# SudhirNikam/cobrix

Hardware: AMD Instinct MI355X
Metric: decoded input GB/s + records/s, fixed-len COMP-3 mix, 1-8 MI355X; % HBM peak (higher is better)
Workload: dtype u8; 1 GPU; SYN200: fixed-length 200-byte EBCDIC records, numeric mix (COMP, COMP-3, zoned DISPLAY overpunch, IBM COMP-2, cp037 X(18)) -- BASELINE config C2; records_per_gpu=50000000, input_bytes_per_gpu=10000000000, job_input_bytes=10000000000, output_columns=28, parallelism=dp1, string_layout=Arrow string views (16 B views + long payloads, one pass), occurs_layout=Arrow lists (present elements only), inputs_resident_in_hbm=True

## Files before the change

cobrix_amd/csrc/cbx_capi.hip:

```cpp
#include <hip/hip_runtime.h>

#include <algorithm>
#include <cstdio>
#include <cstring>
#include <functional>
#include <string>
#include <vector>

#include "cbx_kernels.hip"
#include "cbx_select.h"
#include "cbx_text.h"
#include "cbx_hier.h"
#include "cbx_walk.h"
#include "cbx_chain.h"
#include "cbx_filter.h"
#include "cbx_gather.h"

using namespace cbx;

static thread_local std::string g_err;

static int fail(int code, const std::string& msg) {
    g_err = msg;
    return code;
}

#define HIP_CHECK(x)                                                                   \
    do {                                                                               \
        hipError_t e_ = (x);                                                           \
        if (e_ != hipSuccess) return fail(CBX_E_HIP, std::string(#x) + ": " + hipGetErrorString(e_)); \
    } while (0)

struct cbx_plan {
    std::vector<cbx_field> hfields;
    std::vector<Field> dfields_h;
    std::vector<cbx_array> harrays;
    struct OpSet {
        std::vector<Window> win;
        std::vector<NumOp> nops;
        std::vector<Batch> batches;
        std::vector<StrOp> sops;
        std::vector<GenOp> gops;
        Window* d_win = nullptr;
        NumOp* d_nops = nullptr;
        Batch* d_batches = nullptr;
        StrOp* d_sops = nullptr;
        GenOp* d_gops = nullptr;
        int max_str_items = 0;
        bool has_runs = false;
    } cset, wset;
    bool contig_ok = true;
    int str_stage = 16;
    bool view_staged = false;
    cbx_plan_options opts;
    int n_columns = 0;
    int seg_col = -1;
    int max_pitch = 0;
    int n_seq = 0;
    std::vector<DeferSeq> hdefer;
    std::vector<int32_t> col_is_string;
    std::vector<int32_t> col_slots;
    std::vector<int32_t> col_max_bytes;
    bool view = false;
    bool packed = false;
    std::vector<int32_t> segid_cols;
    std::vector<ListOp> lops;
    ListOp* d_lops = nullptr;
    int32_t* d_list_len = nullptr;  int64_t list_len_cap = 0;
    int32_t* d_list_flag = nullptr; int64_t list_flag_cap = 0;
    Field* d_fields = nullptr;
    DeferSeq* d_defer = nullptr;
    uint64_t* d_defer_bits = nullptr;
    int64_t defer_bits_cap = 0;
    cbx_array* d_arrays = nullptr;
    cbx_segment_map* d_segmap = nullptr;
    uint32_t* d_lut = nullptr;
    DevColumn* d_cols = nullptr;
    std::vector<DevColumn> h_cols;
    std::vector<NumCall> h_ncall;
    std::vector<StrCall> h_scall;
    NumCall* d_ncall = nullptr;
    StrCall* d_scall = nullptr;
    size_t ncall_cap = 0, scall_cap = 0;
    std::vector<int32_t> seq_field, seq_slot;
    std::vector<int64_t> seq_tile_cap;
    std::vector<SeqCall> h_seqcall;
    std::vector<int64_t> h_seq_scratch;
    SeqCall* d_seqcall = nullptr;
    uint32_t* d_str_tot = nullptr;  int64_t str_tot_cap = 0;
    int64_t* d_str_excl = nullptr;  int64_t str_excl_cap = 0;
    int64_t* d_block_sums = nullptr; int64_t block_sums_cap = 0;
    uint32_t* d_local = nullptr;    int64_t local_cap = 0;
    uint8_t* d_scratch = nullptr;   int64_t scratch_cap = 0;
    uint64_t* d_stamps = nullptr;
    int64_t jit_min = 262144;
    bool jit_tried[4 * kPre + 5] = {};
    hipFunction_t jit_fn[4 * kPre + 5] = {};
    bool jit_coop[4 * kPre + 5] = {};
    int rec_extent = 0;
    std::string jit_error;
    int last_kind = 0;
    int32_t* d_status = nullptr;
    int num_cus = 256;
    bool walk = false;
    int32_t walk_root = 0, walk_var = 0, walk_n_handlers = 0, walk_depth = 1, walk_max_rec = 0;
    cbx_walk_node* d_wnodes = nullptr;
    std::vector<cbx_walk_node> h_wnodes;
    std::vector<cbx_walk_array> h_warr;
    bool walk_jit_tried = false;
    hipFunction_t walk_jit_fn = nullptr;
    bool chain_jit_tried = false;
    hipFunction_t chain_jit_fn[5] = {};
    bool last_chain_jit = false;
    cbx_walk_array* d_warr = nullptr;
    cbx_walk_handler* d_whand = nullptr;
    int64_t* d_wslot_base = nullptr;
    int64_t* d_wtile_bytes = nullptr;
    const int64_t* d_rec_base = nullptr;
    const int32_t* d_odo = nullptr;
    int64_t odo_pitch = 0;
    const int64_t* d_dep_seed = nullptr;
    int64_t seed_pitch = 0;
    int32_t seed_root = -1;
    int64_t n_str_slots = 0;
    uint32_t* d_wcursor = nullptr; int64_t wcursor_cap = 0;
    int64_t* d_wvbase = nullptr;
    int32_t* d_wvcol = nullptr;
    int32_t* d_wvslot = nullptr;
    int32_t n_vslots = 0;
    int32_t fid_col = -1, rid_col = -1;
    cbx_plan* pipe_peer = nullptr;
    hipEvent_t pipe_done = nullptr;
    int pipe_count_bpc = 0, pipe_decode_bpc = 0;
    bool profiling = false;
    std::vector<hipEvent_t> ev_pool;
    struct CallEvents { hipEvent_t e[3]; };
    std::vector<CallEvents> ev_calls;
    float flt_ms[3] = {0.f, 0.f, 0.f};
    bool direct_ok = false;
    std::string direct_why;
    std::vector<GatherOp> gather_ops;
    GatherOp* d_gather = nullptr;
// ... 190 lines not shown
        while (e1 < els.size() && std::max(hi, els[e1].eo + els[e1].size) - lo <= wmax && items + (els[e1].str ? 1 : 0) <= kMaxStrItems) {
            hi = std::max(hi, els[e1].eo + els[e1].size);
            items += els[e1].str ? 1 : 0;
            e1++;
        }
        push_window(P, P->wset, std::vector<Elem>(els.begin() + e0, els.begin() + e1), lo, hi, false, {});
        e0 = e1;
    }
    if (!big.empty() || !gen.empty()) push_window(P, P->wset, big, 0, 0, true, gen);
}

template <typename T>
static int upload_vec(T** dst, const std::vector<T>& v) { return upload(dst, v.data(), v.size()); }

static int upload_set(cbx_plan::OpSet& S) {
    int r;
    if ((r = upload_vec(&S.d_win, S.win)) || (r = upload_vec(&S.d_nops, S.nops)) || (r = upload_vec(&S.d_batches, S.batches)) ||
        (r = upload_vec(&S.d_sops, S.sops)) ||
        (r = upload_vec(&S.d_gops, S.gops)))
        return r;
    return CBX_OK;
}

static void free_set(cbx_plan::OpSet& S) {
    (void)hipFree(S.d_win); (void)hipFree(S.d_nops); (void)hipFree(S.d_batches); (void)hipFree(S.d_sops); (void)hipFree(S.d_gops);
}

extern "C" int cbx_plan_create(const cbx_field* fields, int32_t n_fields, const cbx_array* arrays,
                               int32_t n_arrays, const cbx_plan_options* opts, cbx_plan** out_plan) {
    if (!fields || n_fields <= 0 || !opts || !out_plan || n_arrays < 0 || (n_arrays > 0 && !arrays))
        return fail(CBX_E_ARGUMENT, "cbx_plan_create: invalid arguments");
    cbx_plan* P = new cbx_plan();
    P->opts = *opts;
    P->jit_min = opts->jit_min_records < 0 ? -1 : (opts->jit_min_records == 0 ? 262144 : opts->jit_min_records);
    if (const char* e = getenv("CBX_JIT"))
        if (e[0] == '0') P->jit_min = -1;
    P->n_columns = opts->n_columns;
    if (opts->string_views < 0 || opts->string_views > 2)
        { delete P; return fail(CBX_E_ARGUMENT, "cbx_plan_create: string_views must be 0, 1 or 2"); }
    P->view = opts->string_views == 1;
    P->packed = opts->string_views == 2;
    if (P->n_columns <= 0) { delete P; return fail(CBX_E_ARGUMENT, "cbx_plan_create: n_columns must be positive"); }
    P->hfields.assign(fields, fields + n_fields);
    if (n_arrays) P->harrays.assign(arrays, arrays + n_arrays);
    P->col_is_string.assign(P->n_columns, 0);
    P->col_slots.assign(P->n_columns, 1);
    P->col_max_bytes.assign(P->n_columns, 0);

    int lut_max = 1;
    for (int i = 0; i < 256; i++) lut_max = std::max(lut_max, (int)((opts->lut[i] >> 24) & 3));

    for (int i = 0; i < n_fields; i++) {
        const cbx_field& f = fields[i];
        const std::string fi = "field " + std::to_string(i);
        if (f.n_dims < 0 || f.n_dims > CBX_MAX_DIMS) { delete P; return fail(CBX_E_ARGUMENT, fi + ": bad n_dims"); }
        for (int k = 0; k < f.n_dims; k++)
            if (f.dim_count[k] <= 0 || f.dim_array[k] < 0 || f.dim_array[k] >= n_arrays) {
                delete P; return fail(CBX_E_ARGUMENT, fi + ": bad dimension");
            }
        Field d = make_field(f);
        if (f.column < 0 || f.column >= P->n_columns) { delete P; return fail(CBX_E_ARGUMENT, fi + ": bad column"); }
        if (!is_generated(d) && (f.size <= 0 || f.offset < 0)) { delete P; return fail(CBX_E_ARGUMENT, fi + ": bad offset/size"); }
        if (!(f.kind >= CBX_K_STRING && f.kind <= CBX_K_UTF16_LE)) { delete P; return fail(CBX_E_ARGUMENT, fi + ": unknown kind"); }
        if (f.kind == CBX_K_BINARY && f.size > 16) { delete P; return fail(CBX_E_UNSUPPORTED, fi + ": binary wider than 16 bytes"); }
        if (f.kind == CBX_K_ASCII_NUM && (f.size > kAsciiNumMax || f.scale < 0 || f.scale > 100 || f.scale_factor < -100 ||
                                          f.scale_factor > 100)) {
            delete P; return fail(CBX_E_UNSUPPORTED, fi + ": ASCII DISPLAY number wider than 64 bytes");
        }
        if ((f.out_type == CBX_O_DEC64 || f.out_type == CBX_O_DEC128) && (f.out_precision < 1 || f.out_precision > 38)) {
            delete P; return fail(CBX_E_UNSUPPORTED, fi + ": decimal precision outside 1..38");
        }
        if (d.variant == V_STRING) {
            if (f.kind == CBX_K_STRING) d.max_utf8 = lut_max;
            d.seq = P->n_seq;
            P->n_seq += d.n_slots;
            for (int sl = 0; sl < d.n_slots; sl++) {
                P->seq_field.push_back(i);
                P->seq_slot.push_back(sl);
                P->seq_tile_cap.push_back(((int64_t)kWave * f.size * d.max_utf8 + 15) & ~(int64_t)15);
            }
            P->col_max_bytes[f.column] = f.size * d.max_utf8;
        } else if ((d.variant == V_ZONED16 || d.variant == V_GENERIC) && !(f.flags & CBX_F_LIST)) {
            d.defer = (int)P->hdefer.size();
            for (int s = 0; s < d.n_slots; s++) P->hdefer.push_back(DeferSeq{i, s});
        }
        P->dfields_h.push_back(d);
        P->col_is_string[f.column] = is_string_out(f.out_type);
        P->col_slots[f.column] = d.n_slots;
    }
    for (int ai = 0; ai < n_arrays; ai++) {
        const cbx_array& ar = arrays[ai];
        if (ar.dependee >= n_fields || ar.max_count <= 0) { delete P; return fail(CBX_E_ARGUMENT, "array " + std::to_string(ai) + ": bad descriptor"); }
        if (ar.offsets_column >= P->n_columns || (ar.offsets_column >= 0 && (ar.dependee < 0 || ar.n_dims != 0)))
            { delete P; return fail(CBX_E_ARGUMENT, "array " + std::to_string(ai) + ": list layout needs a top-level OCCURS DEPENDING ON"); }
        if (ar.dependee >= 0) {
            const cbx_field& df = fields[ar.dependee];
            if (!(df.flags & CBX_F_INTEGRAL) || df.n_dims != 0 || df.precision > 18)
                { delete P; return fail(CBX_E_UNSUPPORTED, "array " + std::to_string(ai) + ": DEPENDING ON source must be a non-array integral field"); }
        }
    }
    for (int ai = 0; ai < n_arrays; ai++)
        for (int i = 0; i < n_fields; i++) {
            const cbx_field& f = fields[i];
            if (!(f.flags & CBX_F_LIST) || (f.n_dims == 1 && f.dim_array[0] != ai)) continue;
            if (f.n_dims != 1 || arrays[ai].offsets_column < 0 || is_string_out(f.out_type) || f.segment != arrays[ai].segment)
                { delete P; return fail(CBX_E_ARGUMENT, "field " + std::to_string(i) + ": CBX_F_LIST needs a numeric element of a list-layout array in its segment"); }
            ListOp lo{};
            const int16_t none[CBX_MAX_DIMS] = {0, 0, 0, 0};
            lo.op = make_numop(P->dfields_h[i], 0, f.offset, none, none, 0);
            lo.field = i;
            lo.array = ai;
            lo.stride = f.dim_stride[0];
            P->lops.push_back(lo);
        }
    for (ListOp& lo : P->lops) {
        lo.elem_lo = lo.op.eo;
        for (const ListOp& o : P->lops)
            if (o.array == lo.array) lo.elem_lo = std::min(lo.elem_lo, o.op.eo);
    }
    if ((int)P->lops.size() != (int)std::count_if(fields, fields + n_fields, [](const cbx_field& f) { return (f.flags & CBX_F_LIST) != 0; }))
        { delete P; return fail(CBX_E_ARGUMENT, "CBX_F_LIST field outside a list-layout array"); }
    P->seg_col = opts->segment_column;
    if (P->seg_col >= P->n_columns) { delete P; return fail(CBX_E_ARGUMENT, "bad segment column"); }

    int wmax = opts->window_bytes > 0 ? opts->window_bytes : 256;
    if (wmax > kMaxWindowBytes) wmax = kMaxWindowBytes;
    build_contig(P);
    build_windowed(P, wmax);
    int slots = 0;
    if (P->view || P->packed) P->str_stage = 0;
    for (const Field& d : P->dfields_h) {
        if (d.variant != V_STRING) continue;
        const bool fast = d.size <= kStrFastBytes && (d.kind == CBX_K_STRING || d.kind == CBX_K_STRING_ASCII);
        if ((P->view || P->packed) && fast) {
            if (d.max_utf8 > 1 || getenv("CBX_STR_NO_SHIFT")) slots = std::max(slots, kWave * str_lane_slot(d.size, d.max_utf8));
        } else {
            P->str_stage = std::max(P->str_stage, kWave * d.size * d.max_utf8);
            P->view_staged |= P->view;
        }
    }
    P->str_stage = std::min(P->str_stage, kStrStageBytes);
    for (const cbx_field& f : P->hfields) {
        if (f.flags & CBX_F_LIST) continue;
        int64_t e = (int64_t)f.offset + f.size;
        for (int k = 0; k < f.n_dims; k++) e += (int64_t)(f.dim_count[k] - 1) * f.dim_stride[k];
        if (f.kind != CBX_K_RECORD_ID && f.kind != CBX_K_FILE_ID)
            P->rec_extent = std::max(P->rec_extent, (int)std::min<int64_t>(e, 1 << 30));
    }
    P->str_stage = std::max(P->str_stage, slots);

    cbx_segment_map sm = opts->segments;
    if (opts->has_segments) {
        if (sm.n_keys < 0 || sm.n_keys > CBX_MAX_SEG_KEYS || sm.n_levels < 0 || sm.n_levels > CBX_MAX_SEG_LEVELS ||
            sm.prefix_len < 0 || sm.prefix_len > CBX_MAX_SEG_PREFIX || (sm.field_is_int && (sm.field < 0 || sm.field >= n_fields))) {
            delete P; return fail(CBX_E_ARGUMENT, "cbx_plan_create: bad segment map");
        }
        if (sm.field_is_int && !(fields[sm.field].flags & CBX_F_INTEGRAL)) {
            delete P; return fail(CBX_E_UNSUPPORTED, "segment field must be a string or an integral field");
        }
        for (int l = 0; l < sm.n_levels; l++) {
            const int c = sm.level_column[l];
            if (c < 0) continue;
            if (c >= P->n_columns) { delete P; return fail(CBX_E_ARGUMENT, "cbx_plan_create: bad Seg_Id column"); }
            P->col_is_string[c] = 1;
            P->col_slots[c] = 1;
            P->col_max_bytes[c] = sm.prefix_len + 64;
            P->segid_cols.push_back(l);
        }
        for (int k = 0; k < sm.n_keys; k++) {
            std::string u8;
            for (int j = 0; j < opts->segments.key_len[k]; j++) {
// ... 380 lines not shown
    if (mode == 0 && P->packed && P->n_seq > 0 && (contig || span) && P->jit_min >= 0 && c.n_rec >= P->jit_min) {
        const int kp = contig ? contig_kp(sdw) : span_kp;
        const int k = (contig ? 2 : 3) * (kPre + 1) + kp;
        if (!P->jit_tried[k]) {
            P->jit_tried[k] = true;
            std::string err;
            CoopSplit cs;
            P->jit_coop[k] = jit_coop_of(true, span, jit_pro(P), 2, S.win, S.nops, S.batches, S.sops, true, &cs);
            P->jit_fn[k] = jit_get(jit_source(true, kp, jit_pro(P), 2, S.win, S.nops, S.batches, S.sops, span, true),
                                   &err, "cbx_jit_count");
        }
        cfn = P->jit_fn[k];
        ck = k;
    }
    if (mode == 0 && P->packed && P->n_seq > 0 && !cfn && !contig) {
        const int kind = P->last_kind;
        if ((r = launch(P, c, columns, 1, st))) return r;
        P->last_kind = kind;
        if (piped) HIP_CHECK(hipEventRecord(P->pipe_done, st));
    } else if (mode == 0 && P->packed && P->n_seq > 0) {
        KernelArgs ac = a;
        ac.mode = 1;
        size_t clds = lds_own;
        const bool ccoop = cfn && P->jit_coop[ck];
        if (cfn) {
            ac.lds_wave = (a.lds_rows + a.lds_counts + 16 + 15) & ~15;
            clds = 1024 + kLutLds + (ccoop ? (size_t)a.lds_rows + (size_t)kWavesPerBlock * (ac.lds_wave - a.lds_rows)
                                           : (size_t)kWavesPerBlock * ac.lds_wave);
        }
        int cocc = 0;
        const hipError_t ce2 = cfn ? hipModuleOccupancyMaxActiveBlocksPerMultiprocessor(&cocc, cfn, kWave * kWavesPerBlock, clds)
                                   : hipOccupancyMaxActiveBlocksPerMultiprocessor(&cocc, decode_kernel, kWave * kWavesPerBlock, clds);
        int cbpc = (int)std::max<size_t>(1, std::min<size_t>(16, (160 * 1024) / clds));
        if (ce2 == hipSuccess && cocc > 0) cbpc = std::min(cbpc, cocc);
        if (const char* e = getenv("CBX_MAX_BLOCKS_PER_CU")) cbpc = std::max(1, std::min(cbpc, atoi(e)));
        if (piped && P->pipe_count_bpc > 0) cbpc = std::min(cbpc, P->pipe_count_bpc);
        const int64_t cneeded = ccoop ? n_tiles : (n_tiles + kWavesPerBlock - 1) / kWavesPerBlock;
        const int64_t cgrid = std::min<int64_t>(cneeded, (int64_t)P->num_cus * cbpc);
        if (cfn) {
            void* kargs[] = {&ac};
            HIP_CHECK(hipModuleLaunchKernel(cfn, (unsigned)cgrid, 1, 1, kWave * kWavesPerBlock, 1, 1, (unsigned)clds, st, kargs, nullptr));
        } else {
            hipLaunchKernelGGL(decode_kernel, dim3((unsigned)cgrid), dim3(kWave * kWavesPerBlock), clds, st, ac);
            HIP_CHECK(hipGetLastError());
        }
        if ((r = string_scan(P, n_tiles, st))) return r;
        if (piped) HIP_CHECK(hipEventRecord(P->pipe_done, st));
    }
    if (jfn) {
        void* kargs[] = {&a};
        HIP_CHECK(hipModuleLaunchKernel(jfn, (unsigned)grid, 1, 1, kWave * kWavesPerBlock, 1, 1, (unsigned)lds, st, kargs, nullptr));
    } else {
        hipLaunchKernelGGL(decode_kernel, dim3((unsigned)grid), dim3(kWave * kWavesPerBlock), lds, st, a);
        HIP_CHECK(hipGetLastError());
    }
    if (lists) {
        const int64_t lgrid = std::min<int64_t>((n_tiles + kListWaves - 1) / kListWaves, (int64_t)P->num_cus * 8);
        const size_t llds = kListWaves * 2 * (2 * kGuard + kListStage);
        hipFunction_t lfn = nullptr;
        if (P->jit_min >= 0 && c.n_rec >= P->jit_min) {
            const int k = 4 * (kPre + 1);
            if (!P->jit_tried[k]) {
                P->jit_tried[k] = true;
                const std::string src = jit_list_source(P->lops);
                std::string err;
                if (!src.empty()) P->jit_fn[k] = jit_get(src, &err, "cbx_jit_list");
            }
            lfn = P->jit_fn[k];
        }
        const CBX_CONST ListOp* d_lops = (const CBX_CONST ListOp*)P->d_lops;
        int32_t n_lops = (int32_t)P->lops.size();
        if (lfn) {
            void* kargs[] = {&a, &d_lops, &n_lops};
            HIP_CHECK(hipModuleLaunchKernel(lfn, (unsigned)lgrid, 1, 1, kWave * kListWaves, 1, 1, (unsigned)llds, st, kargs, nullptr));
        } else {
            hipLaunchKernelGGL(list_kernel<false>, dim3((unsigned)lgrid), dim3(kWave * kListWaves), llds, st, a, d_lops, n_lops);
        }
        hipLaunchKernelGGL(list_kernel<true>, dim3((unsigned)lgrid), dim3(kWave * kListWaves), llds, st, a,
                           (const CBX_CONST ListOp*)P->d_lops, (int32_t)P->lops.size());
        HIP_CHECK(hipGetLastError());
    }
    if (prof) HIP_CHECK(hipEventRecord(ce.e[1], st));
    if (mode == 0 && n_defer > 0) {
        const unsigned gy = (unsigned)std::min<int64_t>(n_defer, 65535);
        hipLaunchKernelGGL(fixup_kernel, dim3((unsigned)((n_tiles + 4 * kWave - 1) / (4 * kWave)), gy), dim3(4 * kWave), 0, st, a,
                           (const CBX_CONST DeferSeq*)P->d_defer, n_defer);
        HIP_CHECK(hipGetLastError());
    }
    if (P->n_seq > 0 && !((P->view || P->packed) && mode == 0)) {
        if ((r = string_scan(P, n_tiles, st))) return r;
        if (mode == 0) {
            const unsigned gx = (unsigned)((n_tiles + kPlaceWaves * kPlaceTiles - 1) / (kPlaceWaves * kPlaceTiles));
            hipLaunchKernelGGL(str_place_kernel, dim3(gx, (unsigned)std::min<int64_t>(P->n_seq, 65535)), dim3(kWave * kPlaceWaves), 0, st,
                               (const CBX_CONST SeqCall*)P->d_seqcall, (const uint32_t*)P->d_str_tot,
                               (const int64_t*)P->d_str_excl, n_tiles, c.n_rec, P->n_seq, P->d_status);
            HIP_CHECK(hipGetLastError());
        }
    }
    if (prof) {
        HIP_CHECK(hipEventRecord(ce.e[2], st));
        P->ev_calls.push_back(ce);
    }
    return CBX_OK;
}

static std::string field_literal(const Field& f) {
    std::ostringstream o;
    auto arr = [&](const int32_t* v) { o << "{" << v[0] << "," << v[1] << "," << v[2] << "," << v[3] << "}"; };
    o << "{" << f.kind << "," << f.out_type << "," << f.offset << "," << f.size << "," << f.precision << "," << f.scale << ","
      << f.sf << "," << f.out_p << "," << f.out_s << "," << f.flags << "," << f.trim << "," << f.n_dims << ",";
    arr(f.dim_count); o << ","; arr(f.dim_stride); o << ","; arr(f.dim_array);
    o << "," << f.segment << "," << f.column << "," << f.n_slots << "," << f.variant << "," << f.seq << "," << f.max_utf8 << ","
      << f.defer << "," << f.fin << "," << f.plus_null << "," << f.e_mul << "," << f.e_lim << "," << f.lim_lo << "ull," << f.lim_hi
      << "ull}";
    return o.str();
}

struct WalkGen {
    const cbx_plan* P;
    std::ostringstream o;
    int uid = 0, prims = 0;
    bool ok = true;

    void line(int ind, const std::string& t) { o << std::string(2 * ind, ' ') << t << "\n"; }

    void prim(const cbx_walk_node& n, const std::string& off, const std::string& slot, const std::string& m, bool element, int ind) {
        if (n.field < 0) return;
        if (++prims > kJitMaxOps) { ok = false; return; }
        line(ind, "{ constexpr Field f = " + field_literal(P->dfields_h[n.field]) + ";");
        line(ind + 1, "walk_prim_f(a, wl, f, " + std::to_string(n.data_size) + ", " + std::to_string(n.dep_slot) + ", " + off + ", " +
                          slot + ", rec, avail, r, tile, lane, " + m + ", dep, " + (element ? "true" : "false") + "); }");
    }

    void body(int g, const std::string& off, const std::string& slot, const std::string& m, int ind, int depth) {
        if (depth > 64) { ok = false; return; }
        const std::vector<cbx_walk_node>& N = P->h_wnodes;
        for (int c = N[g].child, guard = 0; c >= 0 && ok && guard < (int)N.size(); c = N[c].next, guard++) {
            const cbx_walk_node& n = N[c];
            const std::string K = std::to_string(uid++);
            const bool adv = !(n.flags & CBX_W_REDEFINED);
            if (n.array >= 0) {
                const cbx_array& ar = P->harrays[n.array];
                line(ind, "{   // OCCURS (node " + std::to_string(c) + ")");
                line(ind + 1, "const int cnt" + K + " = " + m + " ? walk_count(a, " + std::to_string(n.array) + ", dep) : 0;");
                if (ar.count_column >= 0) {
                    const std::string cc = std::to_string(ar.count_column);
                    line(ind + 1, "{ const DevColumn cc = ldc(a.cols + " + cc + "); if (" + m + ") *gp((int32_t*)cc.values + (int64_t)(" + slot +
                                      ") * a.pitch + r) = cnt" + K + "; walk_valid(a, wl, cc.validity, " + cc + ", " + slot +
                                      ", tile, lane, " + m + "); }");
                }
                line(ind + 1, "const int cmax" + K + " = (int)wave_max64(cnt" + K + ");");
                line(ind + 1, "int eo" + K + " = " + off + ";");
                line(ind + 1, "for (int e" + K + " = 0; e" + K + " < cmax" + K + "; e" + K + "++) {");
                line(ind + 2, "const bool le" + K + " = " + m + " && e" + K + " < cnt" + K + ";");
                line(ind + 2, "const int s" + K + " = (" + slot + ") * " + std::to_string(std::max(1, ar.max_count)) + " + e" + K + ";");
                if (n.kind == CBX_W_GROUP) {
                    line(ind + 2, "int go" + K + " = eo" + K + ";");
                    body(c, "go" + K, "s" + K, "le" + K, ind + 2, depth + 1);
                    line(ind + 2, "if (le" + K + ") eo" + K + " = go" + K + ";");
                } else {
                    prim(n, "eo" + K, "s" + K, "le" + K, true, ind + 2);
                    line(ind + 2, "if (le" + K + ") eo" + K + " += " + std::to_string(n.data_size) + ";");
                }
                line(ind + 1, "}");
                if (adv)
                    line(ind + 1, "if (" + m + ") " + off + " += " + (P->walk_var ? "eo" + K + " - " + off : std::to_string(n.actual_size)) + ";");
                line(ind, "}");
                continue;
            }
// ... 1798 lines not shown
```

cobrix_amd/csrc/cbx_decode.h:

```cpp
#pragma once
#ifndef __HIPCC_RTC__
#include <hip/hip_runtime.h>
#include <stdint.h>
#endif

#include "cobrix_hip.h"

#define CBX_HD __host__ __device__ __forceinline__
#define CBX_HD_NOINLINE __host__ __device__ __attribute__((noinline))

namespace cbx {

struct U128 {
    uint64_t lo, hi;
};

CBX_HD U128 u128(uint64_t lo, uint64_t hi = 0) { return U128{lo, hi}; }

CBX_HD uint64_t mulhi64(uint64_t a, uint64_t b) {
#if defined(__HIP_DEVICE_COMPILE__)
    return __umul64hi(a, b);
#else
    return (uint64_t)(((unsigned __int128)a * b) >> 64);
#endif
// ... 223 lines not shown
}

template <typename BP>
CBX_HD Val decode_binary(const Field& f, BP p) {
    const int n = f.size;
    const bool be = (f.flags & CBX_F_BIG_ENDIAN) != 0;
    const bool sgn = (f.flags & CBX_F_SIGNED) != 0;
    U128 v = u128(0);
    for (int i = 0; i < n; i++) {
        uint32_t b = p[be ? i : n - 1 - i];
        v.hi = (v.hi << 8) | (v.lo >> 56);
        v.lo = (v.lo << 8) | b;
    }
    bool neg = false;
    if (sgn && n < 16 && n > 0) {
        uint32_t top = p[be ? 0 : n - 1];
        if (top & 0x80) {
            int bits = 8 * n;
            if (bits < 64) {
                v.lo |= ~(uint64_t)0 << bits;
                v.hi = ~(uint64_t)0;
            } else {
                v.hi |= ~(uint64_t)0 << (bits - 64);
            }
            neg = true;
        }
    } else if (sgn && n == 16) {
        neg = (v.hi >> 63) != 0;
    }
    if (f.flags & CBX_F_INTEGRAL) {
        if (n == 1 || n == 2 || n == 4) {
            if (!sgn && n == 4 && (v.lo & 0x80000000u)) return null_val();
            return Val{v.lo, v.hi, true};
        }
        if (n == 8) {
            if (!sgn && (v.lo >> 63)) return null_val();
            return Val{v.lo, (uint64_t)((int64_t)v.lo >> 63), true};
        }
        U128 M = neg ? u128_neg(v) : v;
        return finalize_decimal(M, false, 0, neg, f);
    }
    U128 M = neg ? u128_neg(v) : v;
    if (f.sf == 0) return finalize_decimal(M, false, f.scale, neg, f);
    if (f.sf > 0) {
        bool ok = u128_mul_pow10(M, f.sf);
        return finalize_decimal(M, !ok, 0, neg, f);
    }
    return finalize_decimal(M, false, -f.sf + u128_ndigits(M), neg, f);
}

CBX_HD Val zoned_finish(const Field& f, bool malformed, int sign, int nd, int ndots, int after, U128 D,
                        bool ovf) {
    const bool neg = sign == 2;
    if (malformed || (neg && !(f.flags & CBX_F_SIGNED))) return null_val();
    if (f.flags & CBX_F_INTEGRAL) {
        if (f.precision <= 18) {
            if (ndots != 0 || nd == 0 || ovf || D.hi != 0) return null_val();
            uint64_t lim = f.precision <= 9 ? (neg ? 0x80000000ull : 0x7FFFFFFFull)
                                            : (neg ? 0x8000000000000000ull : 0x7FFFFFFFFFFFFFFFull);
            if (D.lo > lim) return null_val();
            uint64_t v = neg ? (uint64_t)0 - D.lo : D.lo;
            return Val{v, (uint64_t)((int64_t)v >> 63), true};
        }
        if (ndots > 1 || nd == 0) return null_val();
        return finalize_decimal(D, ovf, ndots ? after : 0, neg, f);
    }
    if (f.flags & CBX_F_EXPLICIT_DOT) {
        if (ndots > 1 || nd == 0) return null_val();
        return finalize_decimal(D, ovf, ndots ? after : 0, neg, f);
    }
    if (f.sf == 0) {
        if (ndots != 0 || (sign == 1 && nd < f.scale)) return null_val();
        return finalize_decimal(D, ovf, f.scale, neg, f);
    }
    if (f.sf > 0) {
        if (ndots > 1) return null_val();
        ovf |= !u128_mul_pow10(D, f.sf);
        return finalize_decimal(D, ovf, ndots ? after + f.sf : 0, neg, f);
    }
    if (ndots != 0) return null_val();
    return finalize_decimal(D, ovf, -f.sf + nd, neg, f);
}

template <typename BP>
CBX_HD Val decode_zoned(const Field& f, BP p) {
    const int n = f.size;
    bool malformed = false;
    int sign = 0;
    int nd = 0, ndots = 0, after = 0, sig = 0;
    U128 D = u128(0);
    bool ovf = false;
    for (int i = 0; i < n; i++) {
        uint32_t c = p[i];
        uint32_t hi = c >> 4, lo = c & 15;
        bool dig = lo <= 9 && (hi == 0xF || (sign == 0 && (hi == 0xC || hi == 0xD)));
        bool sch = sign == 0 && (c == 0x60 || c == 0x4E);
        bool dot = c == 0x4B || c == 0x6B;
        bool spc = c == 0x40 || c == 0;
        if (sign == 0 && dig && hi != 0xF) sign = hi == 0xD ? 2 : 1;
        if (sch) sign = c == 0x60 ? 2 : 1;
        malformed |= !(dig || sch || dot || spc);
        if (dig) {
            nd++;
            after += ndots > 0;
            bool s = sig > 0 || lo != 0;
            sig += s;
            if (sig <= 38) u128_muladd(D, 10, lo);
            else ovf = true;
        }
        ndots += dot;
    }
    return zoned_finish(f, malformed, sign, nd, ndots, after, D, ovf);
}

constexpr int kAsciiNumMax = 64;

template <typename BP>
CBX_HD Val ascii_integral(const Field& f, BP p) {
    const int n = f.size;
    int sign = 0, phase = 0, nd = 0;
    bool bad = false, big = false;
    uint64_t v = 0;
    for (int i = 0; i < n; i++) {
        const uint32_t c = p[i];
        if (c == '+' || c == '-') { sign = c == '-' ? 2 : 1; continue; }
        if (c <= 0x20) { phase = phase == 1 ? 2 : phase; continue; }
        if (phase == 2 || c < '0' || c > '9') { bad = true; continue; }
        phase = 1;
        nd++;
        big |= v > 1844674407370955160ull;
        v = v * 10 + (c - '0');
    }
    const bool neg = sign == 2;
    if (bad || nd == 0 || big || (neg && !(f.flags & CBX_F_SIGNED))) return null_val();
    const uint64_t lim = f.precision <= 9 ? (neg ? 0x80000000ull : 0x7FFFFFFFull)
                                          : (neg ? 0x8000000000000000ull : 0x7FFFFFFFFFFFFFFFull);
    if (v > lim) return null_val();
    v = neg ? (uint64_t)0 - v : v;
    return Val{v, (uint64_t)((int64_t)v >> 63), true};
}

CBX_HD Val finalize_decimal_wide(U128 M, int64_t vs, int first_cut, bool neg, const Field& f) {
    const int S = f.out_s;
    if (u128_is_zero(M) && first_cut <= 0) return Val{0, 0, true};
    if (vs == S) {
        if (first_cut >= 5) u128_muladd(M, 1, 1);
        if (!u128_lt(M, U128{f.lim_lo, f.lim_hi})) return null_val();
        const U128 v = neg ? u128_neg(M) : M;
        return Val{v.lo, v.hi, true};
    }
    if (vs < S && S - vs > 38) return null_val();
    if (vs > S && vs - S > 40) return Val{0, 0, true};
    return finalize_decimal(M, false, (int)vs, neg, f);
}

template <typename BP>
CBX_HD Val parse_java_bigdecimal(const Field& f, BP s, int n) {
    int i = 0;
    bool neg = false;
    if (i < n && (s[i] == '+' || s[i] == '-')) { neg = s[i] == '-'; i++; }
    int nd = 0, sig = 0, cut = 0, first_cut = -1;
    bool dot = false;
    int64_t scale = 0;
    U128 M = u128(0);
    for (; i < n; i++) {
        const uint32_t c = s[i];
        if (c >= '0' && c <= '9') {
            nd++;
            scale += dot;
            if (sig > 0 || c != '0') {
                if (sig < 38) { u128_muladd(M, 10, c - '0'); sig++; }
                else { if (cut == 0) first_cut = (int)(c - '0'); cut++; }
            }
        } else if (c == '.' && !dot) {
            dot = true;
        } else if (c == 'e' || c == 'E') {
            i++;
            bool eneg = false;
            if (i < n && (s[i] == '+' || s[i] == '-')) { eneg = s[i] == '-'; i++; }
            if (i >= n) return null_val();
            int64_t ex = 0;
            int ed = 0;
            for (; i < n; i++) {
                if (s[i] < '0' || s[i] > '9') return null_val();
                ex = ex * 10 + (s[i] - '0');
                ed += ex > 0;
                if (ed > 10) return null_val();
            }
            scale -= eneg ? -ex : ex;
            if (scale > 2147483647ll || scale < -2147483648ll) return null_val();
            break;
        } else {
            return null_val();
        }
    }
// ... 644 lines not shown
```

cobrix_amd/csrc/cbx_kernels.hip:

```cpp
#include <hip/hip_runtime.h>

#include "cbx_device.h"
#include "cbx_list.h"

namespace cbx {

struct InterpBody {
    static constexpr int kWords = 0;
    __device__ __forceinline__ void begin(int64_t) {}
    __device__ __forceinline__ void flush(const KernelArgs&, int64_t, int) {}
    __device__ __forceinline__ void post(const KernelArgs&, const TileCtx&, const uint8_t*, uint32_t, const WaveLds&, int,
                                         Stamps&) const {}
    __device__ __forceinline__ void pre(const KernelArgs& a, const TileCtx& t, const uint8_t* img,
                                        uint32_t rec_addr, const WaveLds& l, int lane, Stamps& st) const {
        for (int wi = 0; wi < a.n_windows; wi++) {
            const Window w = ldc(a.windows + wi);
            if (a.mode == 1 && w.sop_begin == w.sop_end) continue;
            if (w.global) {
                decode_generated<false>(a, w, t, lane);
                continue;
            }
#ifdef CBX_STAMPS
            Window ws = w, wn = w;
            ws.batch_begin = ws.batch_end; ws.gen_begin = ws.gen_end;
// ... 127 lines not shown
};

typedef uint32_t u32x4a __attribute__((ext_vector_type(4), aligned(4)));
constexpr int kPlaceWaves = 4;
constexpr int kPlaceTiles = 4;

__global__ __launch_bounds__(kWave * kPlaceWaves) void str_place_kernel(const CBX_CONST SeqCall* seqs, const uint32_t* tot,
                                                                         const int64_t* excl, int64_t n_tiles, int64_t n_rec,
                                                                         int32_t n_seq, int32_t* status) {
    const int lane = threadIdx.x % kWave;
    const int64_t tile0 = ((int64_t)blockIdx.x * kPlaceWaves + threadIdx.x / kWave) * kPlaceTiles;
    if (tile0 >= n_tiles) return;
    for (int seq = blockIdx.y; seq < n_seq; seq += gridDim.y) {
        const SeqCall q = ldc(seqs + seq);
        const int64_t* ex = excl + (int64_t)seq * n_tiles;
        const uint32_t* tt = tot + (int64_t)seq * n_tiles;
        const int64_t seq0 = ex[0];
        const bool pre = 16 * lane + 20 <= q.tile_cap;
        int64_t base[kPlaceTiles];
        uint32_t n[kPlaceTiles], loc[kPlaceTiles], e0[kPlaceTiles];
        u32x4a v0[kPlaceTiles];
#pragma unroll
        for (int u = 0; u < kPlaceTiles; u++) {
            const int64_t tile = tile0 + u < n_tiles ? tile0 + u : n_tiles - 1;
            base[u] = ex[tile] - seq0;
            n[u] = tt[tile];
            loc[u] = gp(q.local)[tile * kWave + lane];
            const CBX_GLOBAL uint32_t* src = gp((const uint32_t*)(q.scratch + tile * (int64_t)q.tile_cap));
            v0[u] = pre ? *(const CBX_GLOBAL u32x4a*)(src + 4 * lane) : u32x4a{0, 0, 0, 0};
            e0[u] = pre ? src[4 * lane + 4] : 0u;
        }
#pragma unroll
        for (int u = 0; u < kPlaceTiles; u++) {
            const int64_t tile = tile0 + u;
            if (tile >= n_tiles) break;
            const int64_t rec = tile * kWave + lane;
            gp(q.offsets)[rec] = q.region + base[u] + loc[u];
            if (tile == n_tiles - 1 && lane == 0) {
                gp(q.offsets)[n_rec] = q.region + base[u] + n[u];
                if (q.size) *gp(q.size) = base[u] + n[u];
            }
            if (base[u] + (int64_t)n[u] > q.capacity) {
                if (lane == 0) atomicOr(status, 1);
                continue;
            }
            const CBX_GLOBAL uint32_t* src = gp((const uint32_t*)(q.scratch + tile * (int64_t)q.tile_cap));
            const CBX_GLOBAL uint8_t* s8 = (const CBX_GLOBAL uint8_t*)src;
            CBX_GLOBAL uint8_t* dst = gp(q.data + base[u]);
            const uint32_t g0 = (uint32_t)((uint64_t)(q.data + base[u]) & 3);
            const uint32_t head = (4 - g0) & 3;
            if (n[u] <= head) {
                if (lane < (int)n[u]) dst[lane] = s8[lane];
                continue;
            }
            const uint32_t ndw = (n[u] - head) >> 2;
            const uint32_t tail = (n[u] - head) & 3;
            if (lane < (int)head) dst[lane] = s8[lane];
            if (lane < (int)tail) dst[head + 4 * ndw + lane] = s8[head + 4 * ndw + lane];
            CBX_GLOBAL uint32_t* d32 = (CBX_GLOBAL uint32_t*)(dst + head);
            const uint32_t sh = head & 3;
            for (uint32_t d = 4u * lane; d < ndw; d += 4u * kWave) {
                u32x4a v = v0[u];
                uint32_t e = e0[u];
                if (d != 4u * lane || !pre) {
                    v = *(const CBX_GLOBAL u32x4a*)(src + d);
                    e = src[d + 4];
                }
                const uint32_t w0 = align_bytes(v.y, v.x, sh), w1 = align_bytes(v.z, v.y, sh);
                const uint32_t w2 = align_bytes(v.w, v.z, sh), w3 = align_bytes(e, v.w, sh);
                if (d + 4 <= ndw) {
                    *(CBX_GLOBAL u32x4a*)(d32 + d) = u32x4a{w0, w1, w2, w3};
                } else {
                    d32[d] = w0;
                    if (d + 1 < ndw) d32[d + 1] = w1;
                    if (d + 2 < ndw) d32[d + 2] = w2;
                }
            }
        }
    }
}

struct DeferSeq {
    int32_t field, slot;
};

__global__ __launch_bounds__(256) void fixup_kernel(KernelArgs a, const CBX_CONST DeferSeq* dseq, int32_t n_defer) {
    const int lane = threadIdx.x % kWave;
    const int64_t tile = ((int64_t)blockIdx.x * (blockDim.x / kWave) + threadIdx.x / kWave) * kWave + lane;
    for (int d = blockIdx.y; d < n_defer; d += gridDim.y) {
        const uint64_t bits = tile < a.n_tiles ? a.defer_bits[(int64_t)d * a.n_tiles + tile] : 0ull;
        uint32_t total;
        const uint32_t ex = wave_excl_scan32((uint32_t)__popcll(bits), lane, total);
        if (total == 0) continue;
        const DeferSeq ds = ldc(dseq + d);
        const CBX_CONST Field* fp = a.fields + ds.field;
        const Field f = ldc(fp);
        int eo = f.offset, rem = ds.slot;
        for (int k = f.n_dims - 1; k >= 0; k--) {
            const int dc = fp->dim_count[k];
            eo += (rem % dc) * fp->dim_stride[k];
            rem /= dc;
        }
        const DevColumn col = ldc(a.cols + f.column);
        for (uint32_t j = lane; j < total + (kWave - 1) - ((total + kWave - 1) % kWave); j += kWave) {
            int lo = 0;
#pragma unroll
            for (int step = kWave / 2; step >= 1; step >>= 1) {
                const uint32_t e = (uint32_t)__shfl((int)ex, lo + step, kWave);
                if (e <= j) lo += step;
            }
            const uint64_t wb = __shfl(bits, lo, kWave);
            const int64_t wt = __shfl(tile, lo, kWave);
            const uint32_t we = (uint32_t)__shfl((int)ex, lo, kWave);
            if (j >= total) continue;
            uint64_t m = wb;
            for (uint32_t r = j - we; r > 0; r--) m &= m - 1;
            const int b = __builtin_ctzll(m);
            const int64_t rec = wt * kWave + b;
            const int64_t base = a.base_shift + (a.rec_off ? a.rec_off[rec] : rec * (int64_t)a.stride);
            const Val x = decode_numeric(f, a.data + base + a.start_off + eo);
            store_value(col, f.out_type, (int64_t)ds.slot * a.pitch + rec, x);
            if (x.valid) atomicOr((unsigned long long*)(col.validity + (int64_t)ds.slot * a.n_tiles + wt), 1ull << b);
        }
    }
}

template <bool kFix>
__global__ __launch_bounds__(kWave * kListWaves) void list_kernel(KernelArgs a, const CBX_CONST ListOp* lops, int32_t n_lops) {
    ListFieldLoop body;
    list_run<kFix>(a, lops, n_lops, body);
}

struct RdwArgs {
    const uint8_t* data;
    int64_t n_bytes;
    cbx_rdw_params p;
};

struct RdwStep {
    int64_t next, off;
    int32_t len;
    bool valid, stop;
    int32_t err;
};

__device__ __forceinline__ uint32_t rdw_header(const RdwArgs& a, int64_t pos) {
    const uintptr_t u = (uintptr_t)(a.data + pos);
    const uint32_t* q = (const uint32_t*)(u & ~(uintptr_t)3);
    if ((const uint8_t*)q + 8 <= a.data + a.n_bytes) return __builtin_amdgcn_alignbyte(q[1], q[0], (uint32_t)(u & 3));
    uint32_t w = 0;
#pragma unroll
    for (int j = 0; j < 4; j++) w |= (uint32_t)a.data[pos + j] << (8 * j);
    return w;
}

__device__ __forceinline__ int64_t rdw_len(const RdwArgs& a, uint32_t h) {
    const uint32_t b0 = h & 0xFF, b1 = (h >> 8) & 0xFF, b2 = (h >> 16) & 0xFF, b3 = h >> 24;
    return (a.p.big_endian ? (int64_t)b1 + 256 * (int64_t)b0 : (int64_t)b2 + 256 * (int64_t)b3) + a.p.adjustment;
}

__device__ __forceinline__ RdwStep rdw_step(const RdwArgs& a, int64_t pos) {
    RdwStep s{0, 0, 0, false, false, 0};
    const int64_t avail = a.n_bytes - pos;
    const int64_t hl = avail < 4 ? avail : 4;
    const int64_t fo = pos + hl;
    int64_t rlen;
    if (a.p.file_header_bytes > 4 && fo == 4) {
        rlen = a.p.file_header_bytes - 4;
    } else if (a.n_bytes > 0 && a.p.file_footer_bytes > 0 && a.n_bytes - fo <= a.p.file_footer_bytes) {
        rlen = a.n_bytes - fo;
    } else if (hl < 4) {
        s.stop = true;
        s.next = a.n_bytes;
        return s;
    } else {
        rlen = rdw_len(a, rdw_header(a, pos));
        if (rlen <= 0) { s.err = -2; return s; }
        if (rlen > 100ll * 1024 * 1024) { s.err = -3; return s; }
        s.valid = true;
    }
    if (rlen <= 0) { s.stop = true; s.next = a.n_bytes; return s; }
    const int64_t rem = a.n_bytes - fo;
    const int64_t got = rlen < rem ? rlen : rem;
    s.off = fo;
    s.len = (int32_t)got;
    s.next = fo + got;
    return s;
}

struct RdwRange {
    int64_t r0, r1;
    int64_t first;
};

struct RdwChunkArgs {
    const RdwRange* ranges;
    int32_t n_ranges;
    int64_t chunk;
    int64_t* entry;
    int64_t* exit_in;
    int64_t* exit_out;
    uint32_t* count;
    int64_t* err;
    int32_t* changed;
    int64_t n;
    uint32_t* stage_off;
// ... 753 lines not shown
```

Before: 2752 GB/s.

## Restructure deferred-field fixup into per-kind kernels with block-wide compaction

Rebuilds the fixup pass that re-decodes deferred zoned/generic fields. Each block now compacts set defer bits across several tile words into a shared-memory index list, and the decoding work is spread over all threads in the block instead of a per-wave binary search and popcount loop. Kernels are templated per field kind and launched per group, which removes the generic decode_numeric dispatch. Zoned fields get a word-aligned windowed byte scan. Element offsets are precomputed on the host. The cost is extra launches, one per kind group, plus extra block syncs, and the fixup only runs on records flagged for deferral.

```diff
diff --git a/cobrix_amd/csrc/cbx_capi.hip b/cobrix_amd/csrc/cbx_capi.hip
--- a/cobrix_amd/csrc/cbx_capi.hip
+++ b/cobrix_amd/csrc/cbx_capi.hip
@@ -58,6 +58,8 @@
     int max_pitch = 0;
     int n_seq = 0;
     std::vector<DeferSeq> hdefer;
+    struct DeferGroup { int kind, begin, count; };
+    std::vector<DeferGroup> defer_groups;
     std::vector<int32_t> col_is_string;
     std::vector<int32_t> col_slots;
     std::vector<int32_t> col_max_bytes;
@@ -414,11 +416,26 @@
             P->col_max_bytes[f.column] = f.size * d.max_utf8;
         } else if ((d.variant == V_ZONED16 || d.variant == V_GENERIC) && !(f.flags & CBX_F_LIST)) {
             d.defer = (int)P->hdefer.size();
-            for (int s = 0; s < d.n_slots; s++) P->hdefer.push_back(DeferSeq{i, s});
+            for (int s = 0; s < d.n_slots; s++) {
+                int eo = d.offset, rem = s;
+                for (int k = d.n_dims - 1; k >= 0; k--) {
+                    eo += (rem % d.dim_count[k]) * d.dim_stride[k];
+                    rem /= d.dim_count[k];
+                }
+                P->hdefer.push_back(DeferSeq{i, s, (int)P->hdefer.size(), eo});
+            }
         }
         P->dfields_h.push_back(d);
         P->col_is_string[f.column] = is_string_out(f.out_type);
         P->col_slots[f.column] = d.n_slots;
+    }
+    std::stable_sort(P->hdefer.begin(), P->hdefer.end(), [&](const DeferSeq& x, const DeferSeq& y) {
+        return P->dfields_h[x.field].kind < P->dfields_h[y.field].kind;
+    });
+    for (int i = 0; i < (int)P->hdefer.size(); i++) {
+        const int kind = P->dfields_h[P->hdefer[i].field].kind;
+        if (P->defer_groups.empty() || P->defer_groups.back().kind != kind) P->defer_groups.push_back({kind, i, 0});
+        P->defer_groups.back().count++;
     }
     for (int ai = 0; ai < n_arrays; ai++) {
         const cbx_array& ar = arrays[ai];
@@ -965,9 +982,8 @@
     }
     if (prof) HIP_CHECK(hipEventRecord(ce.e[1], st));
     if (mode == 0 && n_defer > 0) {
-        const unsigned gy = (unsigned)std::min<int64_t>(n_defer, 65535);
-        hipLaunchKernelGGL(fixup_kernel, dim3((unsigned)((n_tiles + 4 * kWave - 1) / (4 * kWave)), gy), dim3(4 * kWave), 0, st, a,
-                           (const CBX_CONST DeferSeq*)P->d_defer, n_defer);
+        for (const cbx_plan::DeferGroup& g : P->defer_groups)
+            fixup_launch(g.kind, a, (const CBX_CONST DeferSeq*)P->d_defer + g.begin, g.count, st);
         HIP_CHECK(hipGetLastError());
     }
     if (P->n_seq > 0 && !((P->view || P->packed) && mode == 0)) {
diff --git a/cobrix_amd/csrc/cbx_decode.h b/cobrix_amd/csrc/cbx_decode.h
--- a/cobrix_amd/csrc/cbx_decode.h
+++ b/cobrix_amd/csrc/cbx_decode.h
@@ -329,16 +329,13 @@
     return finalize_decimal(D, ovf, -f.sf + nd, neg, f);
 }
 
-template <typename BP>
-CBX_HD Val decode_zoned(const Field& f, BP p) {
-    const int n = f.size;
+struct ZonedScan {
     bool malformed = false;
     int sign = 0;
     int nd = 0, ndots = 0, after = 0, sig = 0;
-    U128 D = u128(0);
+    U128 D{0, 0};
     bool ovf = false;
-    for (int i = 0; i < n; i++) {
-        uint32_t c = p[i];
+    CBX_HD void step(uint32_t c) {
         uint32_t hi = c >> 4, lo = c & 15;
         bool dig = lo <= 9 && (hi == 0xF || (sign == 0 && (hi == 0xC || hi == 0xD)));
         bool sch = sign == 0 && (c == 0x60 || c == 0x4E);
@@ -357,7 +354,18 @@
         }
         ndots += dot;
     }
-    return zoned_finish(f, malformed, sign, nd, ndots, after, D, ovf);
+};
+
+CBX_HD Val zoned_finish(const Field& f, const ZonedScan& z) {
+    return zoned_finish(f, z.malformed, z.sign, z.nd, z.ndots, z.after, z.D, z.ovf);
+}
+
+template <typename BP>
+CBX_HD Val decode_zoned(const Field& f, BP p) {
+    const int n = f.size;
+    ZonedScan z;
+    for (int i = 0; i < n; i++) z.step(p[i]);
+    return zoned_finish(f, z);
 }
 
 constexpr int kAsciiNumMax = 64;
diff --git a/cobrix_amd/csrc/cbx_kernels.hip b/cobrix_amd/csrc/cbx_kernels.hip
--- a/cobrix_amd/csrc/cbx_kernels.hip
+++ b/cobrix_amd/csrc/cbx_kernels.hip
@@ -233,46 +233,126 @@
 
 struct DeferSeq {
     int32_t field, slot;
+    int32_t seq;
+    int32_t eo;
 };
 
-__global__ __launch_bounds__(256) void fixup_kernel(KernelArgs a, const CBX_CONST DeferSeq* dseq, int32_t n_defer) {
-    const int lane = threadIdx.x % kWave;
-    const int64_t tile = ((int64_t)blockIdx.x * (blockDim.x / kWave) + threadIdx.x / kWave) * kWave + lane;
+#ifndef CBX_FIX_WORDS
+#define CBX_FIX_WORDS 4
+#endif
+constexpr int kFixThreads = 256;
+constexpr int kFixWords = CBX_FIX_WORDS;
+constexpr int kFixSpan = kFixThreads * kFixWords;
+constexpr int kFixList = 4096;
+static_assert(kFixSpan * kWave <= 65536, "list entries are 16-bit record indices relative to the span");
+
+template <int NW>
+__device__ __forceinline__ void zoned_scan_window(ZonedScan& z, const CBX_GLOBAL uint8_t* p, int size) {
+    const uint64_t u = (uint64_t)p;
+    const CBX_GLOBAL uint32_t* q = (const CBX_GLOBAL uint32_t*)(u & ~(uint64_t)3);
+    const uint32_t sh = (uint32_t)u & 3u;
+    const uint32_t span = sh + (uint32_t)size;
+    uint32_t d[NW + 1];
+#pragma unroll
+    for (int i = 0; i <= NW; i++) d[i] = 4u * (uint32_t)i < span ? q[i] : 0u;
+    uint32_t w[NW];
+#pragma unroll
+    for (int i = 0; i < NW; i++) w[i] = __builtin_amdgcn_alignbyte(d[i + 1], d[i], sh);
+    for (int i = 0; i < size; i++) {
+        z.step(w[0] & 0xFFu);
+#pragma unroll
+        for (int k = 0; k + 1 < NW; k++) w[k] = __builtin_amdgcn_alignbyte(w[k + 1], w[k], 1u);
+        w[NW - 1] >>= 8;
+    }
+}
+
+template <int KIND>
+__device__ __forceinline__ Val decode_kind(const Field& f, const CBX_GLOBAL uint8_t* p) {
+    if constexpr (KIND == CBX_K_BCD) return decode_bcd(f, p);
+    else if constexpr (KIND == CBX_K_BINARY) return decode_binary(f, p);
+    else if constexpr (KIND == CBX_K_ZONED) {
+#ifdef CBX_FIX_NO_WINDOW
+        return decode_zoned(f, p);
+#else
+        ZonedScan z;
+        if (f.size <= 8) zoned_scan_window<2>(z, p, f.size);
+        else if (f.size <= 12) zoned_scan_window<3>(z, p, f.size);
+        else if (f.size <= 20) zoned_scan_window<5>(z, p, f.size);
+        else for (int i = 0; i < f.size; i++) z.step(p[i]);
+        return zoned_finish(f, z);
+#endif
+    } else return decode_ascii_num(f, p);
+}
+
+template <int KIND>
+__global__ __launch_bounds__(kFixThreads) void fixup_kernel(KernelArgs a, const CBX_CONST DeferSeq* dseq, int32_t n_defer) {
+    __shared__ uint16_t s_list[kFixList];
+    __shared__ uint32_t s_wtot[kFixThreads / kWave];
+    const int tid = threadIdx.x, lane = tid % kWave;
+    const int wid = __builtin_amdgcn_readfirstlane(tid / kWave);
+    const int64_t tile0 = (int64_t)blockIdx.x * kFixSpan;
     for (int d = blockIdx.y; d < n_defer; d += gridDim.y) {
-        const uint64_t bits = tile < a.n_tiles ? a.defer_bits[(int64_t)d * a.n_tiles + tile] : 0ull;
-        uint32_t total;
-        const uint32_t ex = wave_excl_scan32((uint32_t)__popcll(bits), lane, total);
+        if (d != (int)blockIdx.y) __syncthreads();
+        const DeferSeq ds = ldc(dseq + d);
+        const CBX_GLOBAL uint64_t* row = gp(a.defer_bits) + (int64_t)ds.seq * a.n_tiles;
+        uint64_t bits[kFixWords];
+        uint32_t cnt = 0;
+#pragma unroll
+        for (int k = 0; k < kFixWords; k++) {
+            const int64_t tile = tile0 + k * kFixThreads + tid;
+            bits[k] = tile < a.n_tiles ? row[tile] : 0ull;
+            cnt += (uint32_t)__popcll(bits[k]);
+        }
+        uint32_t wtot;
+        uint32_t p = wave_excl_scan32(cnt, lane, wtot);
+        if (lane == 0) s_wtot[wid] = wtot;
+        __syncthreads();
+        uint32_t total = 0;
+#pragma unroll
+        for (int i = 0; i < kFixThreads / kWave; i++) {
+            const uint32_t w = s_wtot[i];
+            p += i < wid ? w : 0u;
+            total += w;
+        }
         if (total == 0) continue;
-        const DeferSeq ds = ldc(dseq + d);
-        const CBX_CONST Field* fp = a.fields + ds.field;
-        const Field f = ldc(fp);
-        int eo = f.offset, rem = ds.slot;
-        for (int k = f.n_dims - 1; k >= 0; k--) {
-            const int dc = fp->dim_count[k];
-            eo += (rem % dc) * fp->dim_stride[k];
-            rem /= dc;
-        }
+        const Field f = ldc(a.fields + ds.field);
         const DevColumn col = ldc(a.cols + f.column);
-        for (uint32_t j = lane; j < total + (kWave - 1) - ((total + kWave - 1) % kWave); j += kWave) {
-            int lo = 0;
-#pragma unroll
-            for (int step = kWave / 2; step >= 1; step >>= 1) {
-                const uint32_t e = (uint32_t)__shfl((int)ex, lo + step, kWave);
-                if (e <= j) lo += step;
-            }
-            const uint64_t wb = __shfl(bits, lo, kWave);
-            const int64_t wt = __shfl(tile, lo, kWave);
-            const uint32_t we = (uint32_t)__shfl((int)ex, lo, kWave);
-            if (j >= total) continue;
-            uint64_t m = wb;
-            for (uint32_t r = j - we; r > 0; r--) m &= m - 1;
-            const int b = __builtin_ctzll(m);
-            const int64_t rec = wt * kWave + b;
-            const int64_t base = a.base_shift + (a.rec_off ? a.rec_off[rec] : rec * (int64_t)a.stride);
-            const Val x = decode_numeric(f, a.data + base + a.start_off + eo);
-            store_value(col, f.out_type, (int64_t)ds.slot * a.pitch + rec, x);
-            if (x.valid) atomicOr((unsigned long long*)(col.validity + (int64_t)ds.slot * a.n_tiles + wt), 1ull << b);
-        }
+        for (uint32_t base = 0; base < total; base += kFixList) {
+            const uint32_t lim = base + kFixList;
+#pragma unroll
+            for (int k = 0; k < kFixWords; k++) {
+                uint64_t m = bits[k];
+                while (m != 0 && p < lim) {
+                    s_list[p - base] = (uint16_t)((uint32_t)(k * kFixThreads + tid) * kWave + (uint32_t)__builtin_ctzll(m));
+                    m &= m - 1;
+                    p++;
+                }
+                bits[k] = m;
+            }
+            __syncthreads();
+            const uint32_t n = total - base < (uint32_t)kFixList ? total - base : (uint32_t)kFixList;
+            for (uint32_t j = tid; j < n; j += kFixThreads) {
+                const uint32_t e = s_list[j];
+                const int64_t wt = tile0 + (e >> 6);
+                const int b = (int)(e & 63);
+                const int64_t rec = wt * kWave + b;
+                const int64_t rbase = a.base_shift + (a.rec_off ? a.rec_off[rec] : rec * (int64_t)a.stride);
+                const Val x = decode_kind<KIND>(f, gp(a.data) + rbase + a.start_off + ds.eo);
+                store_value(col, f.out_type, (int64_t)ds.slot * a.pitch + rec, x);
+                if (x.valid) atomicOr((unsigned long long*)(col.validity + (int64_t)ds.slot * a.n_tiles + wt), 1ull << b);
+            }
+            if (lim < total) __syncthreads();
+        }
+    }
+}
+
+static inline void fixup_launch(int kind, const KernelArgs& a, const CBX_CONST DeferSeq* dseq, int32_t count, hipStream_t st) {
+    const dim3 grid((unsigned)((a.n_tiles + kFixSpan - 1) / kFixSpan), (unsigned)(count < 65535 ? count : 65535));
+    switch (kind) {
+    case CBX_K_BCD: hipLaunchKernelGGL(fixup_kernel<CBX_K_BCD>, grid, dim3(kFixThreads), 0, st, a, dseq, count); break;
+    case CBX_K_BINARY: hipLaunchKernelGGL(fixup_kernel<CBX_K_BINARY>, grid, dim3(kFixThreads), 0, st, a, dseq, count); break;
+    case CBX_K_ZONED: hipLaunchKernelGGL(fixup_kernel<CBX_K_ZONED>, grid, dim3(kFixThreads), 0, st, a, dseq, count); break;
+    default: hipLaunchKernelGGL(fixup_kernel<CBX_K_ASCII_NUM>, grid, dim3(kFixThreads), 0, st, a, dseq, count); break;
     }
 }
 
```

New measurement: 2799 GB/s, median of 6. 1.02x the previous value.
